# hashicorp/consul

Hardware: NVIDIA H100
Metric: million node-ticks/sec (higher is better)
Workload: dtype u32

## Files before the change

### consul_b200/csrc/gs_cuda.cu

```cuda
#include <cuda_runtime.h>
#include <stdio.h>
#include <stdlib.h>
#include <string.h>

#include <map>

#include "gs_aux.h"
#include "gs_backend.h"
#include "gs_query.h"
#include "gs_vmm.h"

#define GS_BLOCK 256
#define GS_GRAPH_TICKS 64
#define GS_WIN_GRAPH 8
#ifndef GS_STRETCH_TICKS
#define GS_STRETCH_TICKS 16
#endif

namespace {

template <bool COORDS>
struct DevSinkT {
  static constexpr bool kCoords = COORDS;
  uint32_t* s_stat;
// ... 53 lines not shown
        "{\n\t.reg .pred p;\n\t"
        "mbarrier.try_wait.parity.shared::cta.b64 p, [%1], %2;\n\t"
        "selp.u32 %0, 1, 0, p;\n\t}"
        : "=r"(done)
        : "r"(gs_smem_addr(bar)), "r"(parity)
        : "memory");
    if (done) return true;
  }
  return false;
}

__device__ __forceinline__ void gs_ranks_wait(const GsDev& d, const GsGlobals& g, uint32_t t) {
  if (threadIdx.x < g.world) {
    uint32_t v;
    do {
      asm volatile("ld.acquire.sys.global.u32 %0, [%1];" : "=r"(v) : "l"(d.tick_flags[g.rank] + threadIdx.x) : "memory");
    } while ((int32_t)(v - t) < 0);
  }
  __syncthreads();
}
__device__ __forceinline__ void gs_ranks_release(const GsDev& d, const GsGlobals& g, uint32_t t_done) {
  __syncthreads();
  if (threadIdx.x == 0u) {
    __threadfence_system();
    const uint32_t arrived = atomicAdd(d.done_ctr, 1u);
    if (arrived == gridDim.x - 1u) {
      __threadfence_system();
      *d.done_ctr = 0u;
      __threadfence_system();
      for (uint32_t r = 0; r < g.world; ++r)
        asm volatile("st.release.sys.global.u32 [%0], %1;" ::"l"(d.tick_flags[r] + g.rank), "r"(t_done) : "memory");
    }
  }
}

__device__ __forceinline__ void gs_q_publish(const GsDev& d, const GsGlobals& g, const uint32_t* s_q, uint32_t t) {
  if (s_q[0] != 0u) {
    if (g.world <= 1u) atomicMax(d.qstate[0] + GS_Q_LAST_ACTIVE, t + 1u);
    else for (uint32_t r = 0; r < g.world; ++r) atomicMax_system(d.qstate[r] + GS_Q_LAST_ACTIVE, t + 1u);
  }
  if (s_q[1] != GS_NEVER) {
    if (g.world <= 1u) atomicMin(d.qstate[0] + GS_Q_HORIZON, s_q[1]);
    else for (uint32_t r = 0; r < g.world; ++r) atomicMin_system(d.qstate[r] + GS_Q_HORIZON, s_q[1]);
  }
}

template <bool COORDS>
__device__ __noinline__ void gs_row_step_impaired_call(const GsDev* dp, const GsGlobals* gp, uint32_t i, uint32_t t,
                                                       uint32_t inb, uint32_t* s_stat, uint32_t* s_heard, uint32_t* s_q) {
  DevSinkT<COORDS> sink{s_stat, s_heard, s_q};
  gs_row_step_body<true>(*dp, *gp, i, t, t % gp->GI, inb, sink);
}
template <bool COORDS>
__device__ __noinline__ void gs_row_step_call(const GsDev* dp, const GsGlobals* gp, uint32_t i, uint32_t t,
                                              uint32_t inb, uint32_t* s_stat, uint32_t* s_heard, uint32_t* s_q) {
  if (dp->imp_loss != nullptr) {
    gs_row_step_impaired_call<COORDS>(dp, gp, i, t, inb, s_stat, s_heard, s_q);
    return;
  }
  DevSinkT<COORDS> sink{s_stat, s_heard, s_q};
  gs_row_step_body<false>(*dp, *gp, i, t, t % gp->GI, inb, sink);
}

struct GsStretchCtl {
  GsStretch out;
  uint32_t violation;
  uint32_t end, floor, depth;
};
__device__ __forceinline__ uint32_t gs_stretch_stop(const GsStretchCtl& c, uint32_t last_active) {
  const uint32_t quiet_at = (last_active > c.floor ? last_active : c.floor) + c.depth;
  return quiet_at < c.end ? quiet_at : c.end;
}

template <bool COORDS>
__global__ void __launch_bounds__(GS_BLOCK, GS_MIN_BLOCKS)
    gs_tick_kernel(const __grid_constant__ GsDev d, const GsGlobals* __restrict__ gp, uint32_t k_off,
                   const GsStretchCtl* __restrict__ stretch) {
  __shared__ uint32_t s_stat[GS_NSTAT * 32];
  __shared__ uint32_t s_heard[32 * 32];
  __shared__ __align__(128) uint32_t s_inb[GS_WARPS][GS_ROUND][GS_TILE];
  __shared__ __align__(128) uint32_t s_due[GS_WARPS][GS_ROUND][GS_TILE];
  __shared__ __align__(8) uint64_t s_bar[GS_WARPS];
  __shared__ uint32_t s_q[2];
  __shared__ uint16_t s_work[GS_WARPS * GS_ROUND * GS_TILE];
  __shared__ uint32_t s_rtile[GS_WARPS];
  __shared__ uint32_t s_wn[2], s_wtake[2];
  static_assert(GS_WARPS <= 8 && GS_ROUND <= 4 && GS_TILE == 128, "s_work entries are 3 + 2 + 7 bits");
  const uint32_t tid = threadIdx.x;
  for (uint32_t x = tid; x < GS_NSTAT * 32u; x += GS_BLOCK) s_stat[x] = 0u;
  for (uint32_t x = tid; x < 32u * 32u; x += GS_BLOCK) s_heard[x] = 0u;
  if (tid == 64u) s_q[0] = 0u;
  if (tid == 65u) s_q[1] = GS_NEVER;
  if (tid >= 66u && tid < 68u) s_wn[tid - 66u] = 0u;
  if (tid >= 68u && tid < 70u) s_wtake[tid - 68u] = 0u;
  if (tid >= 96u && tid < 96u + GS_WARPS) gs_mbar_init(&s_bar[tid - 96u], 1u);
  asm volatile("fence.mbarrier_init.release.cluster;" ::: "memory");
  asm volatile("griddepcontrol.launch_dependents;" ::: "memory");
  asm volatile("griddepcontrol.wait;" ::: "memory");
  if (stretch != nullptr && *d.tick_base + k_off >= gs_stretch_stop(*stretch, __ldcg(d.qstate[0] + GS_Q_LAST_ACTIVE)))
    return;
  __syncthreads();
  const GsGlobals& g = *gp;
  const uint32_t t = *d.tick_base + k_off;
  if (g.world > 1u) gs_ranks_wait(d, g, t);
  const uint32_t cur = t & 1u, P = g.P, pslot = t % P, gslot = t % g.GI;
  const uint32_t pslot_t = (t + P - g.T % P) % P;
  const uint32_t lane = tid & 31u, wib = tid >> 5;
  uint32_t tile_lo = 0, tile_hi = (g.n + GS_TILE - 1u) / GS_TILE;
  if (g.world > 1u) {
    const uint32_t per = g.rows_per_rank / GS_TILE;
    tile_lo = g.rank * per < tile_hi ? g.rank * per : tile_hi;
    tile_hi = tile_lo + per < tile_hi ? tile_lo + per : tile_hi;
  }
  const uint32_t n_warps = gridDim.x * GS_WARPS, n_tiles = tile_hi - tile_lo;
  const uint32_t wid = blockIdx.x * GS_WARPS + wib;
  const uint32_t t_begin = tile_lo + (uint32_t)(((uint64_t)wid * n_tiles) / n_warps);
  const uint32_t t_end = tile_lo + (uint32_t)(((uint64_t)(wid + 1u) * n_tiles) / n_warps);
  const uint32_t* __restrict__ inbox_cur = d.inbox[t & g.ring_mask];
  const bool gated = g.phase_gate != 0u;
  const uint32_t shift = g.phase_shift;
  DevSinkT<COORDS> sink{s_stat, s_heard, s_q};

  const uint32_t max_run = (n_tiles + n_warps - 1u) / n_warps, n_rounds = (max_run + GS_ROUND - 1u) / GS_ROUND;
  bool did_work = false;
  const bool sys_scan = g.world > 1u && (g.flags & 4u);
  auto bring = [&](uint32_t r) {
    const uint32_t b0 = t_begin + r * GS_ROUND < t_end ? t_begin + r * GS_ROUND : t_end;
    const uint32_t b1 = b0 + GS_ROUND < t_end ? b0 + GS_ROUND : t_end;
    const uint32_t tiles = b1 - b0;
    if (!tiles) return;
    uint32_t gate_mask = 0;
    for (uint32_t x = 0; x < tiles; ++x) {
      bool gate = true;
      if (gated) {
        const uint32_t pp = gs_probe_phase(g.rot_p, (b0 + x) >> shift, P);
        gate = pp == pslot || pp == pslot_t;
      }
      gate_mask |= gate ? 1u << x : 0u;
    }
    const size_t off0 = (size_t)b0 * GS_TILE;
    if (sys_scan) {
      for (uint32_t x = 0; x < tiles; ++x) {
        uint4 v;
        asm volatile("ld.relaxed.sys.global.v4.u32 {%0,%1,%2,%3}, [%4];"
                     : "=r"(v.x), "=r"(v.y), "=r"(v.z), "=r"(v.w) : "l"(inbox_cur + off0 + x * GS_TILE + lane * 4u) : "memory");
        *reinterpret_cast<uint4*>(&s_inb[wib][x][lane * 4u]) = v;
        const uint4 dv = (gate_mask >> x) & 1u ? *reinterpret_cast<const uint4*>(d.due + off0 + x * GS_TILE + lane * 4u)
                                               : make_uint4(GS_NEVER, GS_NEVER, GS_NEVER, GS_NEVER);
        *reinterpret_cast<uint4*>(&s_due[wib][x][lane * 4u]) = dv;
      }
      __syncwarp();
      return;
    }
    for (uint32_t x = 0; x < tiles; ++x)
      if (!((gate_mask >> x) & 1u))
        *reinterpret_cast<uint4*>(&s_due[wib][x][lane * 4u]) = make_uint4(GS_NEVER, GS_NEVER, GS_NEVER, GS_NEVER);
    __syncwarp();
    if (lane == 0u) {
      asm volatile("fence.proxy.async.shared::cta;" ::: "memory");
      gs_mbar_expect_tx(&s_bar[wib], (tiles + __popc(gate_mask)) * GS_TILE * 4u);
      gs_bulk_g2s(&s_inb[wib][0][0], inbox_cur + off0, tiles * GS_TILE * 4u, &s_bar[wib]);
      for (uint32_t x = 0; x < tiles; ++x)
        if ((gate_mask >> x) & 1u) gs_bulk_g2s(&s_due[wib][x][0], d.due + off0 + x * GS_TILE, GS_TILE * 4u, &s_bar[wib]);
    }
  };
  bring(0u);
  for (uint32_t round = 0; round < n_rounds; ++round) {
  const uint32_t par = round & 1u;
  const uint32_t r_begin = t_begin + round * GS_ROUND < t_end ? t_begin + round * GS_ROUND : t_end;
  const uint32_t r_end = r_begin + GS_ROUND < t_end ? r_begin + GS_ROUND : t_end;
  if (r_end > r_begin && !sys_scan && !gs_mbar_wait(&s_bar[wib], round & 1u)) {
    if (lane == 0u) atomicExch(d.qstate[g.rank] + GS_Q_VIOLATION, t + 1u);
  }
  for (uint32_t tile = r_begin; tile < r_end; ++tile) {
    const uint32_t st = tile - r_begin;
    uint4 i4 = *reinterpret_cast<const uint4*>(&s_inb[wib][st][lane * 4u]);
    const uint4 d4 = *reinterpret_cast<const uint4*>(&s_due[wib][st][lane * 4u]);
    if (__any_sync(0xFFFFFFFFu, (i4.x | i4.y | i4.z | i4.w) != 0u)) {
      const uint32_t m0 = tile * GS_TILE + lane * 4u;
      const uint4 h4 = __ldcg(reinterpret_cast<const uint4*>(d.heard + m0));
      uint32_t* const w_cur = d.inbox[t & g.ring_mask] + m0;
      uint32_t* const w4 = &i4.x;
      const uint32_t* const h = &h4.x;
      const uint32_t* const du = &d4.x;
      bool stale_any = false;
#pragma unroll
      for (uint32_t u = 0; u < 4u; ++u) {
        const bool pp = g.pp_interval != 0u && gs_pp_due(g.pp_interval, g.rot_pp, (m0 + u) / g.phase_group, t);
        if (w4[u] != 0u && gs_mail_is_stale(g, w4[u], h[u], du[u] == t, pp)) {
          w_cur[u] = 0u;
          s_inb[wib][st][lane * 4u + u] = 0u;
          w4[u] = 0u;
          stale_any = true;
        }
      }
      if (stale_any) sink.activity();
    }
    bool mine = (i4.x | i4.y | i4.z | i4.w) != 0u || d4.x == t || d4.y == t || d4.z == t || d4.w == t;
    bool pp_tile = false;
    if (g.pp_interval != 0u) {
      if (gated) {
        pp_tile = gs_pp_due(g.pp_interval, g.rot_pp, tile >> shift, t);
      } else {
#pragma unroll
        for (uint32_t u = 0; u < 4u; ++u)
          pp_tile |= gs_pp_due(g.pp_interval, g.rot_pp, (tile * GS_TILE + lane * 4u + u) / g.phase_group, t);
      }
      mine |= pp_tile;
    }
    if (__any_sync(0xFFFFFFFFu, mine)) {
      did_work = true;
      __syncwarp();
      const uint32_t base = tile * GS_TILE + lane;
      bool act[4], cand[4];
      bool any_cand = false;
#pragma unroll
      for (int u = 0; u < 4; ++u) {
        const uint32_t w = s_inb[wib][st][u * 32 + lane];
        const bool due_now = s_due[wib][st][u * 32 + lane] == t;
        act[u] = w != 0u || due_now ||
                 (g.pp_interval != 0u && gs_pp_due(g.pp_interval, g.rot_pp, (base + 32u * u) / g.phase_group, t));
        cand[u] = w == 0u && due_now;
        any_cand |= cand[u];
      }
      if (__any_sync(0xFFFFFFFFu, any_cand)) {
        GsFastProbe f[4];
#pragma unroll
        for (int u = 0; u < 4; ++u)
          if (cand[u]) gs_fast_load(d, cur, base + 32u * u, f[u]);
#pragma unroll
        for (int u = 0; u < 4; ++u)
          if (cand[u]) cand[u] = gs_fast_target(d, g, cur, base + 32u * u, f[u]);
        uint32_t n_probe = 0, n_ack = 0;
#pragma unroll
        for (int u = 0; u < 4; ++u) {
          bool acked = false;
          const bool done = cand[u] && gs_fast_finish(d, g, sink, base + 32u * u, t, f[u], &acked);
          if (done) act[u] = false;
          n_probe += __popc(__ballot_sync(0xFFFFFFFFu, done));
          n_ack += __popc(__ballot_sync(0xFFFFFFFFu, done && acked));
        }
        if (lane == 0u && n_probe) {
          atomicAdd(&s_stat[GS_ST_PROBES * 32], n_probe);
          atomicAdd(&s_stat[GS_ST_ACTIVE_ROWS * 32], n_probe);
          if (n_ack) atomicAdd(&s_stat[GS_ST_ACKS * 32], n_ack);
        }
      }
      uint32_t bal[4], n_act = 0;
#pragma unroll
      for (int u = 0; u < 4; ++u) {
        bal[u] = __ballot_sync(0xFFFFFFFFu, act[u]);
        n_act += __popc(bal[u]);
      }
      if (n_act) {
        uint32_t pos = 0;
        if (lane == 0u) pos = atomicAdd(&s_wn[par], n_act);
        pos = __shfl_sync(0xFFFFFFFFu, pos, 0);
        const uint32_t below = (1u << lane) - 1u, key = (wib << 9) | (st << 7) | lane;
#pragma unroll
        for (int u = 0; u < 4; ++u) {
          if (act[u]) s_work[pos + __popc(bal[u] & below)] = (uint16_t)(key | ((uint32_t)u << 5));
          pos += __popc(bal[u]);
        }
      }
    }
  }
  if (lane == 0u) s_rtile[wib] = r_begin;
  __syncwarp();
  if (round + 1u < n_rounds) bring(round + 1u);
  __syncthreads();
  if (tid == 0u) s_wn[par ^ 1u] = s_wtake[par ^ 1u] = 0u;
  const uint32_t n_work = s_wn[par];
  for (;;) {
    uint32_t idx = 0;
    if (lane == 0u) idx = atomicAdd(&s_wtake[par], 32u);
    idx = __shfl_sync(0xFFFFFFFFu, idx, 0);
    if (idx >= n_work) break;
    did_work = true;
    if (idx + lane < n_work) {
      const uint32_t e = s_work[idx + lane];
      const uint32_t i = (s_rtile[e >> 9] + ((e >> 7) & 3u)) * GS_TILE + (e & 127u);
      gs_row_step_call<COORDS>(&d, gp, i, t, __ldcg(inbox_cur + i), s_stat, s_heard, s_q);
    }
  }
  __syncthreads();
  }
  if (g.world > 1u && did_work && !(g.flags & 8u)) __threadfence_system();
  __syncthreads();
  if (tid < GS_NSTAT) {
    uint32_t v = 0;
    for (uint32_t x = 0; x < 32u; ++x) v += s_stat[tid * 32u + ((x + tid) & 31u)];
    if (v) atomicAdd(&d.stats[tid], (unsigned long long)v);
  } else if (tid >= 32u && tid < 32u + GS_MAX_RUMORS) {
    uint32_t r = tid - 32u, c = 0;
    for (uint32_t x = 0; x < 32u; ++x) c += s_heard[r * 32u + ((x + r) & 31u)];
    if (c) {
      uint32_t old = atomicAdd_system(&d.heard_cnt[r], c);
      if (old + c == g.up_count) d.conv_tick[r] = t;
    }
  }
  if (tid == 0u) gs_q_publish(d, g, s_q, t);
  if (g.world > 1u) gs_ranks_release(d, g, t + 1u);
}

template <bool COORDS>
__device__ __noinline__ void gs_window_generic(const GsDev* dp, const GsGlobals* gp, uint32_t gb, uint32_t g_end,
                                               uint32_t tf00, uint32_t tf01, uint32_t tf02, uint32_t tf03,
                                               uint32_t tx00, uint32_t tx01, uint32_t tx02, uint32_t tx03,
                                               uint32_t t0, uint32_t w1, uint32_t* s_stat, uint32_t* s_heard,
                                               uint32_t* s_q, uint32_t* counts) {
  const GsDev& d = *dp;
  const GsGlobals& g = *gp;
  const GsHot h = gs_hot(g);
  const uint32_t P = h.P, T = h.T, lane = threadIdx.x & 31u;
  const uint32_t tf0[4] = {tf00, tf01, tf02, tf03}, tx0[4] = {tx00, tx01, tx02, tx03};
  const bool fast_ok =
      h.loss_thr == 0u && h.graph_n == 0u && d.coord == nullptr && d.imp_loss == nullptr && h.pp_interval == 0u;
  DevSinkT<COORDS> sink{s_stat, s_heard, s_q};
  uint32_t n_probe = 0, n_ack = 0;
  bool did_work = false;
  (void)did_work;
#pragma unroll 1
    for (uint32_t s0 = t0; s0 < w1; s0 += P) {
    const uint32_t off = s0 - t0;
    uint32_t tf[4], tx[4], due[4];
    bool cand[4], slow[4];
    bool any_slow = false;
#pragma unroll
    for (int u = 0; u < 4; ++u) {
      if (gb + u < g_end) {
        tf[u] = tf0[u] + off;
        tx[u] = tx0[u] + off;
        due[u] = __ldcg(d.due + (gb + u) * 32u + lane);
      } else {
        tf[u] = tx[u] = GS_NEVER;
        due[u] = GS_NEVER - 1u;
      }
      cand[u] = fast_ok && due[u] == tf[u] && tf[u] < w1;
      slow[u] = (due[u] == tf[u] && tf[u] < w1 && !fast_ok) || (due[u] == tx[u] && tx[u] < w1);
    }
    GsFastProbe f[4];
#pragma unroll
    for (int u = 0; u < 4; ++u)
      if (cand[u]) gs_fast_load(d, tf[u] & 1u, (gb + u) * 32u + lane, f[u]);
#pragma unroll
    for (int u = 0; u < 4; ++u)
      if (cand[u]) {
        const bool okk = gs_fast_target(d, h, tf[u] & 1u, (gb + u) * 32u + lane, f[u]);
        if (!okk) { cand[u] = false; slow[u] = true; }
      }
#pragma unroll
    for (int u = 0; u < 4; ++u) {
      bool acked = false, done = false;
      if (cand[u]) {
        done = gs_fast_finish(d, h, sink, (gb + u) * 32u + lane, tf[u], f[u], &acked);
        if (!done) slow[u] = true;
        else if (!acked && tf[u] + T < w1) slow[u] = true;
      }
      n_probe += done ? 1u : 0u;
      n_ack += done && acked ? 1u : 0u;
      any_slow |= slow[u];
    }
    if (__any_sync(0xFFFFFFFFu, any_slow)) {
      did_work = true;
#pragma unroll 1
// ... 1613 lines not shown
```

### consul_b200/csrc/gs_row.h

```cpp
#pragma once
#include <string.h>

#include "gs_core.h"
#include "gs_coord.h"

#if defined(__CUDA_ARCH__)
#define GS_DEV __device__ __forceinline__
__device__ __forceinline__ uint32_t gs_atomic_or_sys(uint32_t* p, uint32_t v) {
  uint32_t old;
  asm volatile("atom.global.sys.or.b32 %0, [%1], %2;" : "=r"(old) : "l"(p), "r"(v) : "memory");
  return old;
}
__device__ __forceinline__ uint64_t gs_atomic_min_sys(uint64_t* p, uint64_t v) {
  unsigned long long old;
  asm volatile("atom.global.sys.min.u64 %0, [%1], %2;" : "=l"(old) : "l"(p), "l"((unsigned long long)v) : "memory");
  return old;
}
__device__ __forceinline__ void gs_red_or_sys(uint32_t* p, uint32_t v) {
  asm volatile("red.global.sys.or.b32 [%0], %1;" ::"l"(p), "r"(v) : "memory");
}
#define GS_ATOMIC_OR32(p, v) (g.world > 1u ? gs_atomic_or_sys((p), (v)) : atomicOr((p), (v)))
#define GS_POST_OR32(p, v)                                                         \
  do {                                                                             \
    if (g.world <= 1u) (void)atomicOr((p), (v));                                   \
// ... 255 lines not shown
      if (mode == 1u) {
        if (rank != GS_RANK_ALIVE) continue;
      } else {
        if (rank == GS_RANK_LEFT) continue;
        if (rank == GS_RANK_DEAD && (t - GS_LD_OTHER(&d.change_tick[c])) > g.gtd_ticks) continue;
      }
      if (!gs_knows(d, g, i, c, kc, meta_i)) continue;
      bool dup = false;
      for (uint32_t q = 0; q < cnt; ++q) dup = dup || (out[q] == c);
      if (dup) continue;
      out[cnt++] = c;
    }
  }
  return cnt;
}

GS_DEV uint32_t gs_select_packet(const GsDev& d, const GsGlobals& g, uint32_t i, uint32_t queued) {
  if (g.active_bytes <= g.udp_avail) return queued;
  uint32_t total = 0, qm = queued;
  while (qm) {
#if defined(__CUDA_ARCH__)
    uint32_t r = __ffs(qm) - 1;
#else
    uint32_t r = (uint32_t)__builtin_ctz(qm);
#endif
    qm &= qm - 1;
    total += g.rumors[r].size + (g.rumors[r].qclass ? 3u : 2u);
  }
  if (total <= g.udp_avail) return queued;
  uint32_t used = 0, mask = 0;
  for (uint32_t cls = 0; cls < 3; ++cls) {
    uint32_t cm = queued & g.class_mask[cls];
    const uint32_t ovh = cls ? 3u : 2u;
    while (cm) {
      if (g.udp_avail <= used + ovh) break;
      const uint32_t free_b = g.udp_avail - used - ovh;
      uint32_t best = GS_EMPTY32, best_key = GS_EMPTY32, scan = cm;
      while (scan) {
#if defined(__CUDA_ARCH__)
        uint32_t r = __ffs(scan) - 1;
#else
        uint32_t r = (uint32_t)__builtin_ctz(scan);
#endif
        scan &= scan - 1;
        uint32_t sz = g.rumors[r].size;
        if (sz > free_b) continue;
        uint32_t tx = d.tx[GS_TX(r, g.cap, i)];
        uint32_t key = (tx << 24) | ((0xFFFFu - (sz & 0xFFFFu)) << 8) | (31u - r);
        if (key < best_key) {
          best_key = key;
          best = r;
        }
      }
      if (best == GS_EMPTY32) break;
      mask |= 1u << best;
      cm &= ~(1u << best);
      used += ovh + g.rumors[best].size;
    }
  }
  return mask;
}

template <class Sink>
GS_DEV void gs_log_event(const GsDev& d, const GsGlobals& g, Sink& sink, uint32_t t, uint32_t type,
                         uint32_t subject, uint32_t observer, uint32_t ltime) {
  sink.log_event(d, g, t, type, subject, observer, ltime);
}

GS_DEV bool gs_tile_probe_gate(const GsGlobals& g, uint32_t tile, uint32_t pslot, uint32_t pslot_t) {
  if (!g.phase_gate) return true;
  const uint32_t group = tile >> g.phase_shift;
  const uint32_t pp = gs_probe_phase(g.rot_p, group, g.P);
  return pp == pslot || pp == pslot_t;
}

GS_DEV uint32_t gs_queue_wake_slot(const GsGlobals& g, uint32_t t, uint32_t gslot, uint32_t gphase) {
  const uint32_t next = gslot + 1u == g.GI ? 0u : gslot + 1u;
  const uint32_t delta = (gphase >= next ? gphase - next : gphase + g.GI - next) + 1u;
  return (delta > g.ring_mask + 1u ? t + 1u : t + delta) & g.ring_mask;
}

GS_DEV bool gs_mail_is_stale(const GsGlobals& g, uint32_t w, uint32_t heard, bool due_now, bool pp_now) {
  return (w & (GS_WAKE_BIT | GS_ACC_BIT)) == 0u && !due_now && !pp_now && (w & g.active_mask & ~heard) == 0u;
}

template <bool IMPAIRED, class Sink>
GS_DEV void gs_row_step_body(const GsDev& d, const GsGlobals& g, uint32_t i, uint32_t t, uint32_t gslot,
                             uint32_t inb, Sink& sink) {
  const GsLossCols imp_loss = {IMPAIRED ? d.imp_loss : nullptr, IMPAIRED ? d.imp_recv : nullptr};
  const uint8_t* const imp_delay = IMPAIRED ? d.imp_delay : nullptr;
  const uint8_t* const imp_flags = IMPAIRED ? d.imp_flags : nullptr;
  const uint32_t cur = t & 1u, nxt = cur ^ 1u;
  const uint32_t icur = t & g.ring_mask, inxt = (t + 1u) & g.ring_mask;
  const uint32_t k0 = d.key[cur][i];
  const uint32_t truth = gs_key_truth(k0);
  if (inb != 0u) sink.activity();
  if (truth == GS_TRUTH_NONE) {
    if (inb != 0u) d.inbox[icur][i] = 0u;
    return;
  }
  const uint32_t m0 = d.meta[i];
  const uint32_t due0 = d.due[i];
  const bool up = truth == GS_TRUTH_UP;
  const bool gossip_slot = up && gslot == gs_meta_gphase(m0);
  uint32_t queued = up ? d.queued[i] : 0u;
  const uint32_t rbits = inb & ~(GS_ACC_BIT | GS_WAKE_BIT) & g.active_mask;
  const uint32_t heard0 = rbits != 0u ? d.heard[i] : 0u;
  if (inb != 0u) d.inbox[icur][i] = 0u;
  const bool pp_now = up && g.pp_interval != 0u && gs_pp_due(g.pp_interval, g.rot_pp, i / g.phase_group, t);
  if (inb != 0u && gs_mail_is_stale(g, inb, heard0, due0 == t, pp_now)) return;
  sink.stat(GS_ST_ACTIVE_ROWS, 1);

  if ((inb & ~GS_WAKE_BIT) == 0u && gs_key_rank(k0) == GS_RANK_ALIVE && !(up && due0 == t) &&
      !(gossip_slot && queued != 0u) && !pp_now) {
    if (m0 & GS_META_DIRTY) {
      gs_key_store(d, g, nxt, i, k0);
      d.meta[i] = m0 & ~GS_META_DIRTY;
    }
    if (queued != 0u) gs_post(d, g, sink, gs_queue_wake_slot(g, t, gslot, gs_meta_gphase(m0)), i, GS_WAKE_BIT);
    return;
  }

  uint32_t k = k0, m = m0, due = due0;
  const size_t cap = g.cap;
  uint32_t heard = 0;

  if ((inb & ~GS_WAKE_BIT) != 0u) {
    if ((inb & GS_ACC_BIT) && g.pp_interval != 0u) {
      uint32_t* clk = d.pp_clk + (size_t)cur * 2u * cap;
      const uint32_t cm = GS_LD_OTHER(&clk[i]), ce = GS_LD_OTHER(&clk[cap + i]);
      if (cm | ce) {
        clk[i] = 0u;
        clk[cap + i] = 0u;
        if (up) {
          if (cm > d.ltime_member[i]) d.ltime_member[i] = cm;
          if (ce > d.ltime_event[i]) d.ltime_event[i] = ce;
        }
      }
    }
    if (rbits && up) {
      heard = heard0;
      uint32_t fresh = rbits & ~heard;
      uint32_t accepted = 0;
      while (fresh) {
#if defined(__CUDA_ARCH__)
        uint32_t r = __ffs(fresh) - 1;
#else
        uint32_t r = (uint32_t)__builtin_ctz(fresh);
#endif
        fresh &= fresh - 1;
        const GsRumor& ru = g.rumors[r];
        bool accept = true;
        if (ru.kind == GS_RUMOR_USER_EVENT) {
          uint32_t c = d.ltime_event[i];
          if (ru.ltime >= c) {
            c = ru.ltime + 1u;
            d.ltime_event[i] = c;
          }
          if (ru.ltime < d.event_min[i]) accept = false;
          else if (c > g.event_buffer && ru.ltime < c - g.event_buffer) accept = false;
          if (accept && (m & GS_META_WATCHED))
            gs_log_event(d, g, sink, t, GS_EV_USER, r, i, ru.ltime);
        } else if (ru.kind == GS_RUMOR_JOIN_INTENT || ru.kind == GS_RUMOR_LEAVE_INTENT) {
          uint32_t c = d.ltime_member[i];
          if (ru.ltime >= c) d.ltime_member[i] = ru.ltime + 1u;
        } else if (ru.kind == GS_RUMOR_ALIVE) {
// ... 130 lines not shown
        if (miss > 7u) miss = 7u;
        m = gs_meta_set_nmiss(gs_meta_set_stage(m, GS_STAGE_WAIT_P), miss);
        due = t0 + g.P * (gs_meta_aw(m) + 1u);
      }
      stage = gs_meta_stage(m);
    }
    if (stage == GS_STAGE_WAIT_P && due == t) {
      uint32_t aw = gs_meta_aw(m) + gs_meta_nmiss(m);
      if (aw > g.awareness_max - 1u) aw = g.awareness_max - 1u;
      m = gs_meta_set_stage(gs_meta_set_aw(m, aw), GS_STAGE_IDLE);
      const uint32_t j = d.probe_tgt[i];
      const uint64_t e = ((uint64_t)(~d.probe_inc[i]) << 32) | (uint64_t)i;
      uint64_t* acc = d.acc + (size_t)nxt * GS_K1MAX * cap;
      uint64_t v = e;
      for (uint32_t s = 0; s < GS_K1MAX; ++s) {
        uint64_t old = GS_ATOMIC_MIN64(&acc[(size_t)s * cap + j], v);
        if (old == v || old == GS_EMPTY64) break;
        if (old > v) v = old;
      }
      gs_post(d, g, sink, inxt, j, GS_ACC_BIT);
      sink.stat(GS_ST_PROBE_FAILURES, 1);
      stage = GS_STAGE_IDLE;
    }
    if (stage == GS_STAGE_IDLE && due == t) {
      uint32_t cursor = d.cursor[i], pass = d.pass[i];
      const uint32_t n = gs_peer_count(d, g, i);
      const uint32_t hb = g.graph_n == 0u ? g.perm_bits : gs_perm_bits_of(n);
      GsU4 rk = gs_perm_keys(g.seed_lo, g.seed_hi, i, pass);
      uint32_t checked = 0, target = GS_EMPTY32, ktarget = 0;
      const uint32_t limit = n < GS_PROBE_SKIP_CAP ? n : GS_PROBE_SKIP_CAP;
      while (checked < limit) {
        if (cursor >= n) {
          cursor = 0;
          ++pass;
          ++checked;
          rk = gs_perm_keys(g.seed_lo, g.seed_hi, i, pass);
          continue;
        }
        uint32_t c = gs_peer_at(d, g, i, gs_perm(cursor, n, hb, rk));
        ++cursor;
        uint32_t kc = gs_peer_key(d, cur, c, false);
        uint32_t rank = gs_key_rank(kc);
        if (c == i || gs_key_truth(kc) == GS_TRUTH_NONE || rank == GS_RANK_DEAD ||
            rank == GS_RANK_LEFT || !gs_knows(d, g, i, c, kc, m)) {
          ++checked;
          continue;
        }
        target = c;
        ktarget = kc;
        break;
      }
      d.cursor[i] = cursor;
      d.pass[i] = pass;
      if (target != GS_EMPTY32) {
        sink.stat(GS_ST_PROBES, 1);
        bool ok = gs_key_truth(ktarget) == GS_TRUTH_UP && !gs_lost(g, imp_loss, sink, i, target, t, GS_LK_PING, 0) &&
                  !gs_lost(g, imp_loss, sink, target, i, t, GS_LK_ACK, 0) &&
                  gs_extra(g, imp_delay, i, target) + gs_extra(g, imp_delay, target, i) <= g.T;
        if (ok) {
          uint32_t aw = gs_meta_aw(m);
          m = gs_meta_set_aw(m, aw ? aw - 1u : 0u);
          due = t + g.P;
          sink.stat(GS_ST_ACKS, 1);
          if constexpr (Sink::kCoords) {
            if (d.coord != nullptr) gs_coord_on_ack(d.coord, d.ctag, d.adj, d.adj_idx, imp_delay, g, i, target, t);
          }
        } else {
          m = gs_meta_set_stage(m, GS_STAGE_WAIT_T);
          d.probe_tgt[i] = target;
          d.probe_inc[i] = GS_PEER_INC(d, cur, target, ktarget);
          due = t + g.T;
          sink.horizon(t + g.P);
        }
      } else {
        due = t + g.P;
      }
    }

    if (gossip_slot && queued != 0u) {
      uint32_t peers[8];
      uint32_t kk = g.gossip_nodes > 8u ? 8u : g.gossip_nodes;
      uint32_t np = gs_krandom(d, g, i, t, GS_PUR_GOSSIP, kk, 0u, GS_EMPTY32, m, peers);
      const uint32_t q0 = queued;
      if (g.active_bytes <= g.udp_avail && np != 0u) {
        uint32_t sends[GS_MAX_RUMORS > 8 ? 8 : GS_MAX_RUMORS];
        uint32_t n_pkts = 0, n_q = 0, pm = queued;
        bool few = true;
        while (pm) {
#if defined(__CUDA_ARCH__)
          const uint32_t r = __ffs(pm) - 1;
#else
          const uint32_t r = (uint32_t)__builtin_ctz(pm);
#endif
          pm &= pm - 1;
          if (n_q == 8u) { few = false; break; }
          const uint32_t tx = d.tx[GS_TX(r, cap, i)];
          uint32_t room = g.retransmit_limit > tx ? g.retransmit_limit - tx : 1u;
          if (room == 0u) room = 1u;
          const uint32_t s = room < np ? room : np;
          sends[n_q++] = s;
          if (s > n_pkts) n_pkts = s;
        }
        if (few) {
          pm = queued;
          for (uint32_t x = 0; x < n_q; ++x) {
#if defined(__CUDA_ARCH__)
            const uint32_t r = __ffs(pm) - 1;
#else
            const uint32_t r = (uint32_t)__builtin_ctz(pm);
#endif
            pm &= pm - 1;
            const uint32_t tx = (uint32_t)d.tx[GS_TX(r, cap, i)] + sends[x];
            d.tx[GS_TX(r, cap, i)] = (uint8_t)tx;
            if (tx >= g.retransmit_limit) queued &= ~(1u << r);
            sink.stat(GS_ST_RUMORS_SENT, sends[x]);
          }
          sink.stat(GS_ST_GOSSIP_PACKETS, n_pkts);
          for (uint32_t q = 0; q < n_pkts; ++q) {
            uint32_t pkt = 0;
            pm = q0;
            for (uint32_t x = 0; x < n_q; ++x) {
#if defined(__CUDA_ARCH__)
              const uint32_t r = __ffs(pm) - 1;
#else
              const uint32_t r = (uint32_t)__builtin_ctz(pm);
#endif
              pm &= pm - 1;
              if (sends[x] > q) pkt |= 1u << r;
            }
            if (!gs_lost(g, imp_loss, sink, i, peers[q], t, GS_LK_GOSSIP, q))
              gs_post(d, g, sink, (t + 1u + gs_extra(g, imp_delay, i, peers[q])) & g.ring_mask, peers[q], pkt);
          }
          np = 0u;
        }
      }
      for (uint32_t q = 0; q < np && queued != 0u; ++q) {
        uint32_t pkt = gs_select_packet(d, g, i, queued);
        if (pkt == 0u) break;
        uint32_t pm = pkt;
        while (pm) {
#if defined(__CUDA_ARCH__)
          uint32_t r = __ffs(pm) - 1;
#else
          uint32_t r = (uint32_t)__builtin_ctz(pm);
#endif
          pm &= pm - 1;
          uint32_t tx = (uint32_t)d.tx[GS_TX(r, cap, i)] + 1u;
          d.tx[GS_TX(r, cap, i)] = (uint8_t)tx;
          if (tx >= g.retransmit_limit) queued &= ~(1u << r);
          sink.stat(GS_ST_RUMORS_SENT, 1);
        }
        sink.stat(GS_ST_GOSSIP_PACKETS, 1);
        if (!gs_lost(g, imp_loss, sink, i, peers[q], t, GS_LK_GOSSIP, q))
          gs_post(d, g, sink, (t + 1u + gs_extra(g, imp_delay, i, peers[q])) & g.ring_mask, peers[q], pkt);
      }
      if (queued != q0) d.queued[i] = queued;
    }

    if (pp_now && !(m & GS_META_ISOLATED)) {
      uint32_t partner[1];
      if (gs_krandom(d, g, i, t, GS_PUR_PUSHPULL, 1u, 1u, GS_EMPTY32, m, partner) != 0u) {
        const uint32_t j = partner[0];
        if (!gs_no_tcp(imp_flags, i, j)) {
          uint32_t* req = d.ppreq + (size_t)nxt * GS_PPK * cap;
          uint32_t v = i;
          for (uint32_t s = 0; s < GS_PPK; ++s) {
            const uint32_t old = GS_ATOMIC_MIN32(&req[(size_t)s * cap + j], v);
            if (old == v || old == GS_EMPTY32) break;
            if (old > v) v = old;
          }
          uint32_t* clk = d.pp_clk + (size_t)nxt * 2u * cap;
          GS_ATOMIC_MAX32(&clk[j], d.ltime_member[i]);
          GS_ATOMIC_MAX32(&clk[cap + j], d.ltime_event[i]);
          gs_post(d, g, sink, inxt, j, (d.heard[i] & g.active_mask) | GS_ACC_BIT);
        }
        sink.stat(GS_ST_PUSH_PULLS, 1);
      }
    }
  }

  if (k != k0) {
    gs_key_store(d, g, nxt, i, k);
    m |= GS_META_DIRTY;
  } else if (m0 & GS_META_DIRTY) {
    gs_key_store(d, g, nxt, i, k);
    m &= ~GS_META_DIRTY;
  }
  if (m != m0) d.meta[i] = m;
  if (due != due0) d.due[i] = due;
  if (gs_key_rank(k) == GS_RANK_SUSPECT || (m & GS_META_DIRTY))
    gs_post(d, g, sink, inxt, i, GS_WAKE_BIT);
  else if (queued != 0u)
    gs_post(d, g, sink, gs_queue_wake_slot(g, t, gslot, gs_meta_gphase(m)), i, GS_WAKE_BIT);
}

template <class Sink>
GS_DEV void gs_row_step(const GsDev& d, const GsGlobals& g, uint32_t i, uint32_t t, uint32_t gslot, uint32_t inb,
                        Sink& sink) {
  if (d.imp_loss != nullptr) gs_row_step_body<true>(d, g, i, t, gslot, inb, sink);
  else gs_row_step_body<false>(d, g, i, t, gslot, inb, sink);
}

struct GsFastProbe {
  uint32_t k, m, cursor, pass, c, kc;
};

GS_DEV void gs_fast_load(const GsDev& d, uint32_t cur, uint32_t i, GsFastProbe& f) {
  f.k = d.key[cur][i];
  f.m = d.meta[i];
  f.cursor = d.cursor[i];
  f.pass = d.pass[i];
}

template <class G>
GS_DEV bool gs_fast_target(const GsDev& d, const G& g, uint32_t cur, uint32_t i,
                           GsFastProbe& f) {
  if (g.loss_thr != 0u || g.graph_n != 0u || d.coord != nullptr || d.imp_loss != nullptr)
    return false;
  if (gs_key_truth(f.k) != GS_TRUTH_UP || gs_key_rank(f.k) != GS_RANK_ALIVE) return false;
  if (gs_meta_stage(f.m) != GS_STAGE_IDLE || (f.m & (GS_META_DIRTY | GS_META_ISOLATED))) return false;
  if (f.cursor >= g.n) return false;
  GsU4 rk = gs_perm_keys(g.seed_lo, g.seed_hi, i, f.pass);
  f.c = gs_perm(f.cursor, g.n, g.perm_bits, rk);
  if (f.c == i) return false;
  f.kc = gs_peer_key(d, cur, f.c, false);
  return true;
}

template <class G, class Sink>
GS_DEV bool gs_fast_finish(const GsDev& d, const G& g, Sink& sink, uint32_t i, uint32_t t,
                           const GsFastProbe& f, bool* acked) {
  const uint32_t rank = gs_key_rank(f.kc);
  if (gs_key_truth(f.kc) == GS_TRUTH_NONE || rank == GS_RANK_DEAD || rank == GS_RANK_LEFT ||
      gs_key_pending(f.kc))
    return false;
  if (g.pp_interval != 0u && gs_pp_due(g.pp_interval, g.rot_pp, i / g.phase_group, t))
    return false;
  uint32_t m = f.m;
  if (gs_key_truth(f.kc) == GS_TRUTH_UP && gs_extra(g, nullptr, i, f.c) + gs_extra(g, nullptr, f.c, i) <= g.T) {
    const uint32_t aw = gs_meta_aw(m);
    m = gs_meta_set_aw(m, aw ? aw - 1u : 0u);
    d.due[i] = t + g.P;
    *acked = true;
  } else {
    m = gs_meta_set_stage(m, GS_STAGE_WAIT_T);
    d.probe_tgt[i] = f.c;
    d.probe_inc[i] = GS_PEER_INC(d, t & 1u, f.c, f.kc);
    d.due[i] = t + g.T;
    sink.horizon(t + g.P);
    *acked = false;
  }
  d.cursor[i] = f.cursor + 1u;
  if (m != f.m) d.meta[i] = m;
  return true;
}
```

Before: 740,900.

## Add fast path for gossip-only wake rows with separate candidate work queue

Rows woken only for a gossip turn (wake bit set, no fresh mail, not due) are flagged during the tile scan and pushed to the front of the shared work queue, while other active rows fill it from the back. The worker loop drains candidates first through a specialized gossip routine that picks peers with a single philox block and sends one packet, falling back to the full row step when preconditions fail. The gossip packet logic is also factored into a shared helper that reads tx counters in pairs. This aims to skip the heavy generic row step for the common gossip-only case, at the cost of extra shuffles during the scan, more code, and extra redundant loads when the fast path bails out.

```diff
diff --git a/consul_b200/csrc/gs_cuda.cu b/consul_b200/csrc/gs_cuda.cu
--- a/consul_b200/csrc/gs_cuda.cu
+++ b/consul_b200/csrc/gs_cuda.cu
@@ -159,9 +159,10 @@
   __shared__ __align__(128) uint32_t s_due[GS_WARPS][GS_ROUND][GS_TILE];
   __shared__ __align__(8) uint64_t s_bar[GS_WARPS];
   __shared__ uint32_t s_q[2];
-  __shared__ uint16_t s_work[GS_WARPS * GS_ROUND * GS_TILE];
+  constexpr uint32_t QN = GS_WARPS * GS_ROUND * GS_TILE;
+  __shared__ uint16_t s_work[QN];
   __shared__ uint32_t s_rtile[GS_WARPS];
-  __shared__ uint32_t s_wn[2], s_wtake[2];
+  __shared__ uint32_t s_wn[2], s_wc[2], s_wtake[2];
   static_assert(GS_WARPS <= 8 && GS_ROUND <= 4 && GS_TILE == 128, "s_work entries are 3 + 2 + 7 bits");
   const uint32_t tid = threadIdx.x;
   for (uint32_t x = tid; x < GS_NSTAT * 32u; x += GS_BLOCK) s_stat[x] = 0u;
@@ -170,6 +171,7 @@
   if (tid == 65u) s_q[1] = GS_NEVER;
   if (tid >= 66u && tid < 68u) s_wn[tid - 66u] = 0u;
   if (tid >= 68u && tid < 70u) s_wtake[tid - 68u] = 0u;
+  if (tid >= 70u && tid < 72u) s_wc[tid - 70u] = 0u;
   if (tid >= 96u && tid < 96u + GS_WARPS) gs_mbar_init(&s_bar[tid - 96u], 1u);
   asm volatile("fence.mbarrier_init.release.cluster;" ::: "memory");
   asm volatile("griddepcontrol.launch_dependents;" ::: "memory");
@@ -253,6 +255,7 @@
     const uint32_t st = tile - r_begin;
     uint4 i4 = *reinterpret_cast<const uint4*>(&s_inb[wib][st][lane * 4u]);
     const uint4 d4 = *reinterpret_cast<const uint4*>(&s_due[wib][st][lane * 4u]);
+    uint32_t cv = 0;
     if (__any_sync(0xFFFFFFFFu, (i4.x | i4.y | i4.z | i4.w) != 0u)) {
       const uint32_t m0 = tile * GS_TILE + lane * 4u;
       const uint4 h4 = __ldcg(reinterpret_cast<const uint4*>(d.heard + m0));
@@ -270,8 +273,13 @@
           w4[u] = 0u;
           stale_any = true;
         }
+        if (gs_gossip_candidate(g, w4[u], h[u], du[u] == t, pp)) cv |= 1u << u;
       }
       if (stale_any) sink.activity();
+      cv <<= (lane & 7u) * 4u;
+      cv |= __shfl_xor_sync(0xFFFFFFFFu, cv, 1);
+      cv |= __shfl_xor_sync(0xFFFFFFFFu, cv, 2);
+      cv |= __shfl_xor_sync(0xFFFFFFFFu, cv, 4);
     }
     bool mine = (i4.x | i4.y | i4.z | i4.w) != 0u || d4.x == t || d4.y == t || d4.z == t || d4.w == t;
     bool pp_tile = false;
@@ -323,21 +331,31 @@
           if (n_ack) atomicAdd(&s_stat[GS_ST_ACKS * 32], n_ack);
         }
       }
-      uint32_t bal[4], n_act = 0;
+      const bool any_gt = __any_sync(0xFFFFFFFFu, cv != 0u);
+      uint32_t bal[4], balc[4], n_act = 0, n_c = 0;
 #pragma unroll
       for (int u = 0; u < 4; ++u) {
-        bal[u] = __ballot_sync(0xFFFFFFFFu, act[u]);
+        balc[u] = any_gt ? __shfl_sync(0xFFFFFFFFu, cv, u * 8) : 0u;
+        bal[u] = __ballot_sync(0xFFFFFFFFu, act[u]) & ~balc[u];
         n_act += __popc(bal[u]);
-      }
-      if (n_act) {
-        uint32_t pos = 0;
-        if (lane == 0u) pos = atomicAdd(&s_wn[par], n_act);
+        n_c += __popc(balc[u]);
+      }
+      if (n_act | n_c) {
+        uint32_t pos = 0, pc = 0;
+        if (lane == 0u) {
+          if (n_act) pos = atomicAdd(&s_wn[par], n_act);
+          if (n_c) pc = atomicAdd(&s_wc[par], n_c);
+        }
         pos = __shfl_sync(0xFFFFFFFFu, pos, 0);
+        pc = __shfl_sync(0xFFFFFFFFu, pc, 0);
         const uint32_t below = (1u << lane) - 1u, key = (wib << 9) | (st << 7) | lane;
 #pragma unroll
         for (int u = 0; u < 4; ++u) {
-          if (act[u]) s_work[pos + __popc(bal[u] & below)] = (uint16_t)(key | ((uint32_t)u << 5));
+          const uint16_t e = (uint16_t)(key | ((uint32_t)u << 5));
+          if ((balc[u] >> lane) & 1u) s_work[pc + __popc(balc[u] & below)] = e;
+          else if (act[u]) s_work[QN - 1u - pos - __popc(bal[u] & below)] = e;
           pos += __popc(bal[u]);
+          pc += __popc(balc[u]);
         }
       }
     }
@@ -346,18 +364,22 @@
   __syncwarp();
   if (round + 1u < n_rounds) bring(round + 1u);
   __syncthreads();
-  if (tid == 0u) s_wn[par ^ 1u] = s_wtake[par ^ 1u] = 0u;
-  const uint32_t n_work = s_wn[par];
+  if (tid == 0u) s_wn[par ^ 1u] = s_wc[par ^ 1u] = s_wtake[par ^ 1u] = 0u;
+  const uint32_t n_work = s_wn[par], n_cand = s_wc[par], c_end = (n_cand + 31u) & ~31u;
   for (;;) {
     uint32_t idx = 0;
     if (lane == 0u) idx = atomicAdd(&s_wtake[par], 32u);
     idx = __shfl_sync(0xFFFFFFFFu, idx, 0);
-    if (idx >= n_work) break;
+    if (idx >= c_end + n_work) break;
     did_work = true;
-    if (idx + lane < n_work) {
-      const uint32_t e = s_work[idx + lane];
+    const bool cand = idx < c_end;
+    const uint32_t x = cand ? idx + lane : idx - c_end + lane;
+    if (x < (cand ? n_cand : n_work)) {
+      const uint32_t e = s_work[cand ? x : QN - 1u - x];
       const uint32_t i = (s_rtile[e >> 9] + ((e >> 7) & 3u)) * GS_TILE + (e & 127u);
-      gs_row_step_call<COORDS>(&d, gp, i, t, __ldcg(inbox_cur + i), s_stat, s_heard, s_q);
+      const uint32_t inb = __ldcg(inbox_cur + i);
+      if (!(cand && gs_gossip_turn(d, g, sink, i, t, gslot)))
+        gs_row_step_call<COORDS>(&d, gp, i, t, inb, s_stat, s_heard, s_q);
     }
   }
   __syncthreads();
diff --git a/consul_b200/csrc/gs_row.h b/consul_b200/csrc/gs_row.h
--- a/consul_b200/csrc/gs_row.h
+++ b/consul_b200/csrc/gs_row.h
@@ -361,6 +361,78 @@
 
 GS_DEV bool gs_mail_is_stale(const GsGlobals& g, uint32_t w, uint32_t heard, bool due_now, bool pp_now) {
   return (w & (GS_WAKE_BIT | GS_ACC_BIT)) == 0u && !due_now && !pp_now && (w & g.active_mask & ~heard) == 0u;
+}
+
+GS_DEV bool gs_gossip_candidate(const GsGlobals& g, uint32_t w, uint32_t heard, bool due_now, bool pp_now) {
+  return (w & (GS_WAKE_BIT | GS_ACC_BIT)) == GS_WAKE_BIT && !due_now && !pp_now && (w & g.active_mask & ~heard) == 0u;
+}
+
+GS_DEV bool gs_queued_tx(const GsDev& d, const GsGlobals& g, uint32_t i, uint32_t queued, uint64_t* txs) {
+  uint64_t v = 0;
+  uint32_t n_q = 0, pm = queued;
+  while (pm) {
+#if defined(__CUDA_ARCH__)
+    const uint32_t p = (uint32_t)(__ffs(pm) - 1) >> 1;
+    const uint32_t pair = *reinterpret_cast<const uint16_t*>(d.tx + GS_TX(2u * p, g.cap, i));
+#else
+    const uint32_t p = (uint32_t)__builtin_ctz(pm) >> 1;
+    uint16_t pair16;
+    memcpy(&pair16, d.tx + GS_TX(2u * p, g.cap, i), 2);
+    const uint32_t pair = pair16;
+#endif
+    const uint32_t two = (pm >> (2u * p)) & 3u;
+    pm &= ~(3u << (2u * p));
+    if (n_q + (two & 1u) + (two >> 1) > 8u) return false;
+    if (two & 1u) v |= (uint64_t)(pair & 0xFFu) << (8u * n_q++);
+    if (two & 2u) v |= (uint64_t)(pair >> 8) << (8u * n_q++);
+  }
+  *txs = v;
+  return true;
+}
+
+template <class Sink, class Peer>
+GS_DEV uint32_t gs_gossip_one_packet(const GsDev& d, const GsGlobals& g, Sink& sink, const GsLossCols& loss,
+                                     const uint8_t* delay, uint32_t i, uint32_t t, uint32_t queued, uint64_t txs,
+                                     uint32_t np, Peer peer) {
+  const size_t cap = g.cap;
+  auto sends = [&](uint32_t x) {
+    const uint32_t tx = (uint32_t)(txs >> (8u * x)) & 0xFFu;
+    const uint32_t room = g.retransmit_limit > tx ? g.retransmit_limit - tx : 1u;
+    return room < np ? room : np;
+  };
+  uint32_t left = queued, pm = queued, n_pkts = 0, sent = 0;
+  for (uint32_t x = 0; pm; ++x) {
+#if defined(__CUDA_ARCH__)
+    const uint32_t r = __ffs(pm) - 1;
+#else
+    const uint32_t r = (uint32_t)__builtin_ctz(pm);
+#endif
+    pm &= pm - 1;
+    const uint32_t s = sends(x), tx = ((uint32_t)(txs >> (8u * x)) & 0xFFu) + s;
+    d.tx[GS_TX(r, cap, i)] = (uint8_t)tx;
+    if (tx >= g.retransmit_limit) left &= ~(1u << r);
+    sent += s;
+    if (s > n_pkts) n_pkts = s;
+  }
+  sink.stat(GS_ST_RUMORS_SENT, sent);
+  sink.stat(GS_ST_GOSSIP_PACKETS, n_pkts);
+  for (uint32_t q = 0; q < n_pkts; ++q) {
+    uint32_t pkt = 0;
+    pm = queued;
+    for (uint32_t x = 0; pm; ++x) {
+#if defined(__CUDA_ARCH__)
+      const uint32_t r = __ffs(pm) - 1;
+#else
+      const uint32_t r = (uint32_t)__builtin_ctz(pm);
+#endif
+      pm &= pm - 1;
+      if (sends(x) > q) pkt |= 1u << r;
+    }
+    const uint32_t j = peer(q);
+    if (!gs_lost(g, loss, sink, i, j, t, GS_LK_GOSSIP, q))
+      gs_post(d, g, sink, (t + 1u + gs_extra(g, delay, i, j)) & g.ring_mask, j, pkt);
+  }
+  return left;
 }
 
 template <bool IMPAIRED, class Sink>
@@ -657,57 +729,11 @@
       uint32_t kk = g.gossip_nodes > 8u ? 8u : g.gossip_nodes;
       uint32_t np = gs_krandom(d, g, i, t, GS_PUR_GOSSIP, kk, 0u, GS_EMPTY32, m, peers);
       const uint32_t q0 = queued;
-      if (g.active_bytes <= g.udp_avail && np != 0u) {
-        uint32_t sends[GS_MAX_RUMORS > 8 ? 8 : GS_MAX_RUMORS];
-        uint32_t n_pkts = 0, n_q = 0, pm = queued;
-        bool few = true;
-        while (pm) {
-#if defined(__CUDA_ARCH__)
-          const uint32_t r = __ffs(pm) - 1;
-#else
-          const uint32_t r = (uint32_t)__builtin_ctz(pm);
-#endif
-          pm &= pm - 1;
-          if (n_q == 8u) { few = false; break; }
-          const uint32_t tx = d.tx[GS_TX(r, cap, i)];
-          uint32_t room = g.retransmit_limit > tx ? g.retransmit_limit - tx : 1u;
-          if (room == 0u) room = 1u;
-          const uint32_t s = room < np ? room : np;
-          sends[n_q++] = s;
-          if (s > n_pkts) n_pkts = s;
-        }
-        if (few) {
-          pm = queued;
-          for (uint32_t x = 0; x < n_q; ++x) {
-#if defined(__CUDA_ARCH__)
-            const uint32_t r = __ffs(pm) - 1;
-#else
-            const uint32_t r = (uint32_t)__builtin_ctz(pm);
-#endif
-            pm &= pm - 1;
-            const uint32_t tx = (uint32_t)d.tx[GS_TX(r, cap, i)] + sends[x];
-            d.tx[GS_TX(r, cap, i)] = (uint8_t)tx;
-            if (tx >= g.retransmit_limit) queued &= ~(1u << r);
-            sink.stat(GS_ST_RUMORS_SENT, sends[x]);
-          }
-          sink.stat(GS_ST_GOSSIP_PACKETS, n_pkts);
-          for (uint32_t q = 0; q < n_pkts; ++q) {
-            uint32_t pkt = 0;
-            pm = q0;
-            for (uint32_t x = 0; x < n_q; ++x) {
-#if defined(__CUDA_ARCH__)
-              const uint32_t r = __ffs(pm) - 1;
-#else
-              const uint32_t r = (uint32_t)__builtin_ctz(pm);
-#endif
-              pm &= pm - 1;
-              if (sends[x] > q) pkt |= 1u << r;
-            }
-            if (!gs_lost(g, imp_loss, sink, i, peers[q], t, GS_LK_GOSSIP, q))
-              gs_post(d, g, sink, (t + 1u + gs_extra(g, imp_delay, i, peers[q])) & g.ring_mask, peers[q], pkt);
-          }
-          np = 0u;
-        }
+      uint64_t txs;
+      if (g.active_bytes <= g.udp_avail && np != 0u && gs_queued_tx(d, g, i, queued, &txs)) {
+        queued = gs_gossip_one_packet(d, g, sink, imp_loss, imp_delay, i, t, queued, txs, np,
+                                      [&](uint32_t q) { return peers[q]; });
+        np = 0u;
       }
       for (uint32_t q = 0; q < np && queued != 0u; ++q) {
         uint32_t pkt = gs_select_packet(d, g, i, queued);
@@ -829,3 +855,61 @@
   if (m != f.m) d.meta[i] = m;
   return true;
 }
+
+template <class Sink>
+GS_DEV bool gs_gossip_turn(const GsDev& d, const GsGlobals& g, Sink& sink, uint32_t i, uint32_t t, uint32_t gslot) {
+  if (g.graph_n != 0u || d.imp_loss != nullptr || g.active_bytes > g.udp_avail) return false;
+  const uint32_t cur = t & 1u;
+  const uint32_t k0 = d.key[cur][i], m = d.meta[i], queued = d.queued[i];
+  const uint32_t n = g.n;
+  const uint32_t tries = (3u * n > GS_KR_MAX_TRIES || n > 0x55555555u) ? GS_KR_MAX_TRIES : 3u * n;
+  const GsU4 blk = gs_philox(g.seed_lo, g.seed_hi, i, t, GS_PUR_GOSSIP, 0u);
+  uint32_t cc[4], kc[4];
+#pragma unroll
+  for (uint32_t x = 0; x < 4u; ++x) {
+    cc[x] = gs_fastmod(gs_u4_get(blk, x), n, g.n_magic);
+    kc[x] = (x < tries && cc[x] != i) ? gs_peer_key(d, cur, cc[x], false) : 0u;
+  }
+  uint64_t txs = 0;
+  const bool few = gs_queued_tx(d, g, i, queued, &txs);
+  const uint32_t kk = g.gossip_nodes > 8u ? 8u : g.gossip_nodes;
+  if (gs_key_truth(k0) != GS_TRUTH_UP || gs_key_rank(k0) != GS_RANK_ALIVE || gs_key_pending(k0) ||
+      gs_meta_stage(m) != GS_STAGE_IDLE || (m & (GS_META_DIRTY | GS_META_ISOLATED)) || gslot != gs_meta_gphase(m) ||
+      queued == 0u || !few || kk == 0u)
+    return false;
+  uint32_t took = 0, np = 0;
+#pragma unroll
+  for (uint32_t x = 0; x < 4u; ++x) {
+    if (!(x < tries && np < kk)) continue;
+    const uint32_t c = cc[x];
+    if (c == i || gs_key_truth(kc[x]) == GS_TRUTH_NONE) continue;
+    const uint32_t rank = gs_key_rank(kc[x]);
+    if (rank == GS_RANK_LEFT) continue;
+    if (rank == GS_RANK_DEAD || gs_key_pending(kc[x])) return false;
+    bool dup = false;
+#pragma unroll
+    for (uint32_t y = 0; y < x; ++y) dup = dup || (((took >> y) & 1u) && cc[y] == c);
+    if (dup) continue;
+    took |= 1u << x;
+    ++np;
+  }
+  if (np < kk) return false;
+  sink.activity();
+  d.inbox[t & g.ring_mask][i] = 0u;
+  sink.stat(GS_ST_ACTIVE_ROWS, 1);
+  const GsLossCols no_loss = {nullptr, nullptr};
+  const uint32_t left = gs_gossip_one_packet(d, g, sink, no_loss, nullptr, i, t, queued, txs, np, [&](uint32_t q) {
+    uint32_t c = 0, seen = 0;
+#pragma unroll
+    for (uint32_t x = 0; x < 4u; ++x) {
+      if ((took >> x) & 1u) {
+        if (seen == q) c = cc[x];
+        ++seen;
+      }
+    }
+    return c;
+  });
+  if (left != queued) d.queued[i] = left;
+  if (left != 0u) gs_post(d, g, sink, gs_queue_wake_slot(g, t, gslot, gs_meta_gphase(m)), i, GS_WAKE_BIT);
+  return true;
+}
```

Result: faster. 834,100 (median of 6 runs) (+12.6%).
